# imironhead/ml_super_resolution

Measured on AMD Instinct MI355X. Metric: VDSR-20 training patches/sec (41x41, batch 256 per GPU); fwd HR megapixels/sec alongside, higher is better.
Workload: dtype f32; 1 GPU; BASELINE configs[2]: VDSR 20-layer 3x3x64 residual, RGB, batch 256x41x41 per GPU, fwd+bwd+TF-Adam, random-init weights; global_batch=256, patch=41, parallelism=dp1

## Files before the change

include/srx.h:

```cpp
#ifndef SRX_H_
#define SRX_H_

#include <stddef.h>
#include <stdint.h>

#ifdef __cplusplus
extern "C" {
#endif

typedef void* srx_stream_t;

typedef enum {
    SRX_OK = 0,
    SRX_ERR_BAD_ARG = -1,
    SRX_ERR_UNSUPPORTED = -2,
    SRX_ERR_WORKSPACE = -3,
    SRX_ERR_LAUNCH = -4,
    SRX_ERR_ALIGN = -5
} srx_status;

typedef enum { SRX_PAD_SAME = 0, SRX_PAD_VALID = 1 } srx_pad_mode;

typedef enum {
    SRX_ACT_NONE = 0,
// ... 18 lines not shown
} srx_conv_desc;

const char* srx_version(void);
const char* srx_last_error(void);

int srx_set_conv_path(int pipelined);

int srx_set_wgrad_path(int path);

int srx_conv_chain(const srx_conv_desc* d, int op, int in_act, int layers, const float* const* x, const float* const* w,
                   const float* const* bias, const float* const* aux, float* const* y, srx_stream_t stream);

int srx_conv_chain_supported(const srx_conv_desc* d, int op, int in_act);

int srx_set_chain(int on);

int srx_conv2d_precision_supported(const srx_conv_desc* d, int op);

size_t srx_conv2d_workspace_bytes(const srx_conv_desc* d, int op);

int srx_conv2d_fwd(const srx_conv_desc* d, const float* x, const float* w, const float* bias,
                   const float* skip, float* y, void* ws, size_t ws_bytes, srx_stream_t stream);

int srx_conv2d_bwd_data(const srx_conv_desc* d, const float* dpre, const float* w,
                        const float* x_in, int in_act, float* dx_out, void* ws, size_t ws_bytes,
                        srx_stream_t stream);

int srx_conv2d_bwd_data_acc(const srx_conv_desc* d, const float* dpre, const float* w, const float* dx_acc,
                            float* dx_out, void* ws, size_t ws_bytes, srx_stream_t stream);

// ... 163 lines not shown
```

ml_super_resolution_amd/_lib.py:

```python
import ctypes
import os

_HERE = os.path.dirname(os.path.abspath(__file__))
LIB_PATH = os.path.join(_HERE, 'libsrx.so')

SRX_OK = 0
PAD_SAME, PAD_VALID = 0, 1
ACT_NONE, ACT_RELU, ACT_TANH, ACT_LRELU, ACT_SIGMOID = 0, 1, 2, 3, 4
OP_FWD, OP_BWD_DATA, OP_BWD_FILTER = 0, 1, 2
PRECISION_FP32, PRECISION_BF16X3 = 0, 1
PRECISION_BY_NAME = {'highest': PRECISION_FP32, 'high': PRECISION_BF16X3}

ACT_BY_NAME = {None: ACT_NONE, 'none': ACT_NONE, 'relu': ACT_RELU, 'tanh': ACT_TANH,
               'lrelu': ACT_LRELU, 'leaky_relu': ACT_LRELU, 'sigmoid': ACT_SIGMOID}
PAD_BY_NAME = {'same': PAD_SAME, 'valid': PAD_VALID}

EXPORTS = [
    'srx_version', 'srx_last_error', 'srx_set_conv_path', 'srx_set_wgrad_path', 'srx_set_chain', 'srx_conv_chain', 'srx_conv_chain_supported', 'srx_conv2d_precision_supported', 'srx_conv2d_workspace_bytes', 'srx_conv2d_fwd',
    'srx_conv2d_bwd_data', 'srx_conv2d_bwd_filter', 'srx_conv2d_bwd_filter_partials', 'srx_conv2d_bwd_filter_reduce', 'srx_act_bwd', 'srx_depth_to_space',
    'srx_space_to_depth', 'srx_stream_copy', 'srx_mse_fwd_bwd', 'srx_l2_loss', 'srx_reduce_scratch_bytes',
    'srx_adam_tf_step', 'srx_adam_tf_step_dev', 'srx_momentum_clip_step', 'srx_rownorm_loss_fwd_bwd', 'srx_psnr', 'srx_ssim', 'srx_ssim_scratch_bytes', 'srx_saturate_u8', 'srx_affine', 'srx_u8_to_unit_float', 'srx_gaussian_blur', 'srx_resize_bilinear',
    'srx_upsample_nearest', 'srx_upsample_nearest_bwd', 'srx_add_relu_grad',
    'srx_conv2d_bwd_data_acc', 'srx_conv3x3_blocked', 'srx_conv3x3_blocked_bwd_filter_workspace_bytes', 'srx_conv3x3_blocked_bwd_filter',
    'srx_conv3x3_blocked_ex', 'srx_conv3x3_blocked_bwd_filter_ex_workspace_bytes', 'srx_conv3x3_blocked_bwd_filter_ex',
    'srx_espcn_forward', 'srx_espcn_forward_keep', 'srx_debug_poison_lds', 'srx_srcnn_forward', 'srx_maxpool2x2', 'srx_maxpool2x2_bwd', 'srx_maxpool2x2_bwd_masked', 'srx_subsample2', 'srx_subsample2_bwd',
    'srx_channel_blocks_to_nhwc', 'srx_nhwc_to_channel_blocks', 'srx_channel_normalize', 'srx_channel_normalize_bwd',
    'srx_extract_patches16', 'srx_texture_gram', 'srx_texture_gram_bwd', 'srx_pil_resample_ksize', 'srx_pil_resample_coeffs', 'srx_resample_u8', 'srx_u8_to_pm1', 'srx_log_loss', 'srx_vgg_preprocess', 'srx_add_scaled', 'srx_resize_bicubic_tf', 'srx_column_sums', 'srx_gemm_workspace_bytes', 'srx_gemm',
]


class SrxError(RuntimeError):
    pass

# ... 22 lines not shown
    if not os.path.exists(LIB_PATH):
        raise SrxError('libsrx.so not found at %s -- build it with `make -C %s` (or '
                       '__graft_entry__.build()); there is no CPU fallback' %
                       (LIB_PATH, os.path.join(_HERE, 'csrc')))
    import torch
    L = ctypes.CDLL(LIB_PATH)
    vp, sz, i, f = ctypes.c_void_p, ctypes.c_size_t, ctypes.c_int, ctypes.c_float
    dp = ctypes.POINTER(ConvDesc)
    L.srx_version.restype = ctypes.c_char_p
    L.srx_last_error.restype = ctypes.c_char_p
    L.srx_set_conv_path.argtypes = [i]
    L.srx_set_wgrad_path.argtypes = [i]
    L.srx_set_chain.argtypes = [i]
    L.srx_conv_chain_supported.argtypes = [dp, i, i]
    L.srx_conv_chain.argtypes = [dp, i, i, i, vp, vp, vp, vp, vp, vp]
    L.srx_conv2d_precision_supported.argtypes = [dp, i]
    L.srx_conv2d_workspace_bytes.argtypes = [dp, i]
    L.srx_conv2d_workspace_bytes.restype = sz
    L.srx_reduce_scratch_bytes.restype = sz
    L.srx_conv2d_fwd.argtypes = [dp, vp, vp, vp, vp, vp, vp, sz, vp]
    L.srx_conv2d_bwd_data.argtypes = [dp, vp, vp, vp, i, vp, vp, sz, vp]
    L.srx_conv2d_bwd_filter.argtypes = [dp, vp, vp, vp, vp, vp, f, vp, sz, vp]
    L.srx_conv2d_bwd_filter_partials.argtypes = [dp, vp, vp, vp, sz, ctypes.POINTER(ctypes.c_int), vp]
    L.srx_conv2d_bwd_filter_reduce.argtypes = [dp, vp, i, vp, vp, vp, f, vp]
    L.srx_act_bwd.argtypes = [vp, vp, vp, sz, i, vp]
    L.srx_depth_to_space.argtypes = [vp, vp, i, i, i, i, i, vp]
    L.srx_space_to_depth.argtypes = [vp, vp, i, i, i, i, i, vp]
    L.srx_stream_copy.argtypes = [vp, vp, sz, vp]
    L.srx_mse_fwd_bwd.argtypes = [vp, vp, sz, f, vp, i, vp, vp, vp]
    L.srx_l2_loss.argtypes = [vp, vp, sz, f, vp, i, vp, vp]
# ... 63 lines not shown
```

ml_super_resolution_amd/csrc/conv_kernels.hip.h:

```cpp
#pragma once
#include <hip/hip_runtime.h>
#include <stdint.h>
#include <type_traits>

namespace srx {

typedef float f32x4 __attribute__((ext_vector_type(4)));

enum { ACT_NONE = 0, ACT_RELU = 1, ACT_TANH = 2, ACT_LRELU = 3, ACT_SIGMOID = 4 };

struct ConvArgs {
    const float* x;
    const float* w;
    const float* bias;
    const float* skip;
    const float* mask;
    float* y;
    int N, H, W, OH, OW, Cin, Cout;
    int pad_t, pad_l;
    int TH, TW, NTX, RS;
    int units_total;
    int act, post_relu, mask_act;
    float inv_rs;
    int stagger;
// ... 15 lines not shown
    int units_total;
    float inv_rs;
    int stagger;
    int zero_slot;
    int stride;
    unsigned long long* trace;
};

constexpr int kChainMax = 32;
struct ChainPtrs {
    const float* x[kChainMax];
    const float* w[kChainMax];
    const float* bias[kChainMax];
    const float* aux[kChainMax];
    float* y[kChainMax];
    int L;
};

template <int CINP>
struct Lds {
    static constexpr int PS = (CINP == 4) ? 4 : CINP + 4;
};

__device__ __forceinline__ float srx_tanhf(float x) {
    const float ax = fabsf(x);
    const float x2 = ax * ax;
    float p = fmaf(x2, -0.006274174898862839f, 0.021071631461381912f);
    p = fmaf(x2, p, -0.053852297365665436f);
    p = fmaf(x2, p, 0.13332585990428925f);
    p = fmaf(x2, p, -0.33333316445350647f);
// ... 2396 lines not shown
        }
    }
    bsum += __shfl_xor(bsum, 16);
    bsum += __shfl_xor(bsum, 32);
    if (qpart == 0 && kq == 0 && co_ok) pw[(size_t)TAPS * a.Cin * a.Cout + co] = bsum;
}

template <int IMM>
__device__ __forceinline__ float dpre_fire_imm(__amdgpu_buffer_rsrc_t rsrc, int voff, int soff) {
    float b;
    asm volatile("buffer_load_dword %0, %1, %2, %3 offen offset:%4" : "=&a"(b) : "v"(voff), "s"(rsrc), "s"(soff), "n"(IMM) : "memory");
    return b;
}

template <int KH, int KW, int CINP, int NCH, int OWC>
__global__ __launch_bounds__(256, 1) void wgrad_rows_full_kernel(const WgradArgs a) {
    extern __shared__ __attribute__((aligned(16))) float lds[];
    constexpr int PS = Lds<CINP>::PS;
    constexpr int TAPS = KH * KW;
    constexpr int ROWS = TAPS * CINP;
    constexpr int Q = (ROWS + 63) / 64;
    constexpr int NQP = 4 / NCH;
    constexpr int QW = (Q + NQP - 1) / NQP;
    constexpr int TPP = CINP / 4, PPP = 256 / TPP;
    constexpr int SPR = OWC / 4;
    constexpr int THC = 3;
    constexpr int RSZ = OWC + 1;
    constexpr int COUTC = 64;
    constexpr int U = THC * SPR + 1;
    constexpr int JP = (RSZ + PPP - 1) / PPP;
    constexpr int NPASSES = (THC + KH - 1) * JP;
// ... 17 lines not shown
    char* ldsb = reinterpret_cast<char*>(lds);
    const int buf_bytes = (a.zero_slot + 4) * PS * 4;

    typedef __attribute__((address_space(3))) const f32x4 lds_f32x4;
    const int lds_base = (int)(uintptr_t)(__attribute__((address_space(3))) char*)ldsb;
    int xw[QW];
#pragma unroll
    for (int k = 0; k < QW; ++k) {
        const int q = qpart + k * NQP;
        int R = 64 * q + 4 * li;
        if (q >= Q || R >= ROWS) R = 0;
        const int tap = R / CINP, ci = R % CINP;
        xw[k] = lds_base + ((kq + (tap / KW) * RSZ + (tap % KW)) * PS + ci) * 4;
    }
    const int dX = kq * (RSZ - 1) * PS * 4;
    {
        const f32x4 z = {0.f, 0.f, 0.f, 0.f};
        for (int i = tid; i < 2 * buf_bytes / 16; i += 256) reinterpret_cast<f32x4*>(lds)[i] = z;
    }
    const int voff_lane = tid * 16;
    const int wl_lane = (sp * PS + 4 * c4) * 4;
    StageGeo SG;
    SG.JP1 = __builtin_amdgcn_readfirstlane(JP - 1);
    SG.rowfix_g = __builtin_amdgcn_readfirstlane((a.W - JP * PPP) * CINP * 4);
    SG.rowfix_l = __builtin_amdgcn_readfirstlane((RSZ - JP * PPP) * PS * 4);
    SG.m_first = uniform64(__ballot(sp >= a.pad_l));
    SG.m_last = uniform64(__ballot((JP - 1) * PPP + sp < RSZ));
    SG.m_row = SG.m_last; SG.m_mid = ~0ull;
    const int colb = 16 * COUTC;
    const int lane_b = (kq * COUTC + co_c) * 4;
    const int vb0 = lane_b, vb1 = lane_b + 4 * colb, vb2 = lane_b + 8 * colb;
// ... 181 lines not shown
#pragma unroll
        for (int g = 0; g < 4; ++g) {
#pragma unroll
            for (int r = 0; r < 4; ++r) {
                const int R = 64 * q + 4 * (4 * kq + r) + g;
                const int tap = R / CINP, ci = R % CINP;
                if (R < ROWS && ci < a.Cin && co_ok) pw[((size_t)tap * a.Cin + ci) * a.Cout + co] = acc[k][g][r];
            }
        }
    }
    bsum += __shfl_xor(bsum, 16);
    bsum += __shfl_xor(bsum, 32);
    if (qpart == 0 && kq == 0 && co_ok) pw[(size_t)TAPS * a.Cin * a.Cout + co] = bsum;
}

}
```

ml_super_resolution_amd/csrc/launchers.h:

```cpp
#pragma once
#include "conv_kernels.hip.h"

namespace srx {

struct ConvKey {
    int kh, kw, cinp, nch;
    bool wt;
};

bool launch_conv_k3c64(const ConvKey& k, const ConvArgs& a, int grid, size_t lds, hipStream_t s, hipError_t* err);
bool launch_conv_k3c32(const ConvKey& k, const ConvArgs& a, int grid, size_t lds, hipStream_t s, hipError_t* err);
bool launch_conv_c4(const ConvKey& k, const ConvArgs& a, int grid, size_t lds, hipStream_t s, hipError_t* err);
bool launch_conv_misc(const ConvKey& k, const ConvArgs& a, int grid, size_t lds, hipStream_t s, hipError_t* err);
bool launch_pipe_k3c64(const ConvKey& k, const ConvArgs& a, int grid, size_t lds, hipStream_t s, hipError_t* err);
bool launch_pipe_other(const ConvKey& k, const ConvArgs& a, int grid, size_t lds, hipStream_t s, hipError_t* err);
bool launch_wgrad_narrow(const ConvKey& k, const WgradArgs& a, int grid, hipStream_t s, hipError_t* err);
bool launch_conv_narrow(const ConvKey& k, const ConvArgs& a, hipStream_t s, hipError_t* err);
bool launch_conv_1x1(const ConvKey& k, const ConvArgs& a, long min_pixels, hipStream_t s, hipError_t* err);
bool launch_conv_rows3x3(const ConvKey& k, const ConvArgs& a, long min_pixels, hipStream_t s, hipError_t* err);
bool launch_conv_pack3(const ConvKey& k, const ConvArgs& a, long min_pixels, hipStream_t s, hipError_t* err);
bool launch_conv_kwrows(const ConvKey& k, const ConvArgs& a, long min_pixels, hipStream_t s, hipError_t* err);
bool launch_pipe_strip(const ConvKey& k, const ConvArgs& a, int grid, size_t lds, hipStream_t s, hipError_t* err);
bool launch_conv_generic(const ConvKey& k, const ConvArgs& a, int grid, size_t lds, hipStream_t s, hipError_t* err);
bool launch_wgrad(const ConvKey& k, const WgradArgs& a, int grid, size_t lds, hipStream_t s, hipError_t* err);
// ... 2 lines not shown
bool launch_wgrad_lin_pack3(const ConvKey& k, const WgradArgs& a, int grid, size_t lds, hipStream_t s, hipError_t* err);
bool launch_wgrad_lin_strip(const ConvKey& k, const WgradArgs& a, int grid, size_t lds, hipStream_t s, hipError_t* err);
bool launch_wgrad_pipe(const ConvKey& k, const WgradArgs& a, int grid, size_t lds, hipStream_t s, hipError_t* err);
bool launch_wgrad_kwcols(const ConvKey& k, const WgradArgs& a, int max_partials, long min_pixels, int* n_partials, hipStream_t s, hipError_t* err);
bool launch_wgrad_1x1(const ConvKey& k, const WgradArgs& a, int max_partials, int* n_partials, hipStream_t s, hipError_t* err);
bool launch_wgrad_rows_full(const ConvKey& k, const WgradArgs& a, int grid, size_t lds, hipStream_t s, hipError_t* err);
bool launch_wgrad_rows_strip(const ConvKey& k, const WgradArgs& a, int grid, size_t lds, hipStream_t s, hipError_t* err);
bool launch_wgrad_lin_pairs(const ConvKey& k, const WgradPairs& q, int grid, int pairs, bool strips, size_t lds, hipStream_t s, hipError_t* err);

__attribute__((weak)) hipError_t launch_conv_chain(bool wt, bool aux, const ConvArgs& a, const ChainPtrs& c, int grid, size_t lds, hipStream_t s);

hipError_t launch_reduce_partials(const float* part, int G, int stride, int wn, int cout, float* dw, float* dbias,
                                  const float* w, float wd, hipStream_t s);
hipError_t launch_reduce_partials_pairs(const float* part, int G, int stride, int wn, int cout, float* dw, float* dbias,
                                        int pairs, int cob, hipStream_t s);

template <typename K, typename A>
inline hipError_t launch_with_lds(K kernel, const A& a, int grid, size_t lds, hipStream_t s, int grid_y = 1) {
    static thread_local const void* configured[64];
    static thread_local int n_configured = 0;
    const void* fn = reinterpret_cast<const void*>(kernel);
    bool known = false;
    for (int i = 0; i < n_configured; ++i) known |= (configured[i] == fn);
    if (!known) {
        hipError_t e = hipFuncSetAttribute(fn, hipFuncAttributeMaxDynamicSharedMemorySize, 160 * 1024);
        if (e != hipSuccess) return e;
        if (n_configured < 64) configured[n_configured++] = fn;
    }
    hipLaunchKernelGGL(kernel, dim3(grid, grid_y), dim3(256), lds, s, a);
    return hipGetLastError();
// ... 93 lines not shown
```

ml_super_resolution_amd/csrc/srx_api.hip:

```cpp
#include <math.h>
#include <stdarg.h>
#include <atomic>
#include <stdio.h>
#include <stdlib.h>
#include <string.h>

#include "../../include/srx.h"
#include "elementwise.h"
#include "launchers.h"
#include "bf16x3.h"

using namespace srx;

namespace {

thread_local char g_err[512] = "";

struct Knobs {
    int pipe_default, narrow, wgrad_lin, wgrad_pipe, wgrad_pipe_strip, wgrad_rows_full, wgrad_1x1, wgrad_pack3, kwrows_min_pixels, big_route_min_pixels, strip_d2s, conv_1x1_min_pixels, pack3_dgrad;
    int chain;
    unsigned long long* trace;
    int dbg;
};
int env_int(const char* name, int dflt) { const char* e = getenv(name); return e ? atoi(e) : dflt; }
Knobs read_knobs() {
    Knobs k;
    k.pipe_default = env_int("SRX_PIPE", 1);
    k.narrow = env_int("SRX_NARROW", 1);
    k.wgrad_lin = env_int("SRX_WGRAD_LIN", 1);
    k.wgrad_pipe = env_int("SRX_WGRAD_PIPE", 1);
    k.wgrad_pipe_strip = env_int("SRX_WGRAD_PIPE_STRIP", 1);
    k.kwrows_min_pixels = env_int("SRX_KWROWS_MIN_PIXELS", 4096);
    k.big_route_min_pixels = env_int("SRX_BIG_ROUTE_MIN_PIXELS", 60000);
    k.conv_1x1_min_pixels = env_int("SRX_CONV_1X1_MIN_PIXELS", 100000);
    k.pack3_dgrad = env_int("SRX_PACK3_DGRAD", 1);
    k.strip_d2s = env_int("SRX_STRIP_D2S", 1);
    k.wgrad_rows_full = env_int("SRX_WGRAD_ROWS_FULL", 1);
    k.wgrad_1x1 = env_int("SRX_WGRAD_1X1", 1);
    k.wgrad_pack3 = env_int("SRX_WGRAD_PACK3", 1);
    k.chain = env_int("SRX_CHAIN", 1);
    k.trace = nullptr;
    k.dbg = 0;
#ifdef SRX_TRACE
    { const char* tp = getenv("SRX_TRACE_PTR"); k.trace = tp ? (unsigned long long*)strtoull(tp, nullptr, 0) : nullptr; }
    k.dbg = env_int("SRX_DBG", 0);
#endif
    return k;
}
const Knobs& knobs() { static const Knobs k = read_knobs(); return k; }

std::atomic<int> g_use_pipe{-1};
std::atomic<int> g_chain{-1};
int use_chain() { const int v = g_chain.load(std::memory_order_relaxed); return v < 0 ? (knobs().chain ? 1 : 0) : v; }
int use_pipe() { const int v = g_use_pipe.load(std::memory_order_relaxed); return v < 0 ? knobs().pipe_default : v; }
std::atomic<int> g_wgrad_path{-1};
int wgrad_path_default() { return !knobs().wgrad_lin ? 0 : ((knobs().wgrad_pipe || knobs().wgrad_pipe_strip) ? 2 : 1); }
int wgrad_path() { const int v = g_wgrad_path.load(std::memory_order_relaxed); return v < 0 ? wgrad_path_default() : v; }

int cu_count() {
    static std::atomic<int> cached[64];
    int dev = 0;
    if (hipGetDevice(&dev) != hipSuccess || dev < 0 || dev >= 64) { (void)hipGetLastError(); return 256; }
    int n = cached[dev].load(std::memory_order_relaxed);
    if (n > 0) return n;
    if (hipDeviceGetAttribute(&n, hipDeviceAttributeMultiprocessorCount, dev) != hipSuccess || n <= 0) {
        (void)hipGetLastError();
        n = 256;
    }
// ... 519 lines not shown
    memset(&a, 0, sizeof(a));
    a.x = dpre; a.w = w; a.bias = nullptr; a.skip = dx_acc; a.mask = x_in; a.y = dx_out;
    fill_conv_args(&a, p, d->N, OH, OW, d->Cout, d->Cin);
    a.act = SRX_ACT_NONE; a.post_relu = 0; a.mask_act = in_act;
    return dispatch_conv(p, true, a, (hipStream_t)stream);
}

static void wgrad_tile_for_linear_walk(const srx_conv_desc* d, Plan* p) {
    if (p->NTX != 1 || wgrad_path() < 1) return;
    const size_t slot_bytes = (size_t)((p->cinp == 4) ? 4 : p->cinp + 4) * 4;
    while (p->TH > 1 && p->lds_bytes + 4 * slot_bytes > 80 * 1024) {
        p->TH -= 1;
        p->lds_bytes = ((size_t)(p->TH + d->KH - 1) * p->RS + (d->KW - 1)) * slot_bytes;
    }
}

int srx_conv2d_bwd_filter_partials(const srx_conv_desc* d, const float* x, const float* dpre, void* ws, size_t ws_bytes,
                                   int* n_partials, srx_stream_t stream) {
    int rc = check_desc(d);
    if (rc) return rc;
    if (!x || !dpre || !n_partials) return fail(SRX_ERR_BAD_ARG, "null tensor pointer");
    if (!aligned16(x) || !aligned16(dpre)) return fail(SRX_ERR_ALIGN, "tensor base pointers must be 16-byte aligned");
    if (d->precision == SRX_PRECISION_BF16X3) {
        if ((rc = bf16x3_supported(d, SRX_OP_BWD_FILTER)) != SRX_OK) return rc;
        Bf3Plan bp;
        bf16x3_plan(d->N, d->H, d->W, max_grid(), true, &bp);
        const size_t need = (size_t)bp.grid * part_stride(d) * sizeof(float);
        if (!ws || ws_bytes < need) return fail(SRX_ERR_WORKSPACE, "bwd_filter needs %zu workspace bytes, got %zu", need, ws_bytes);
        if (!aligned16(ws)) return fail(SRX_ERR_ALIGN, "workspace must be 16-byte aligned");
        const hipError_t err = launch_wgrad3x3c64_bf16x3(x, dpre, (float*)ws, (int)part_stride(d), d->N, d->H, d->W, bp, (hipStream_t)stream);
// ... 35 lines not shown
    const bool lin_ok = use_lin && p.NTX == 1 && OW >= 4 && p.RS >= 8 && p.RS == d->W + pl && (long)p.TH * OW * d->Cout * 4 < (1L << 30) &&
                        (long)d->H * d->W * d->Cin * 4 < (1L << 31) - 4096;
    const size_t lin_lds = p.lds_bytes + 4 * (size_t)((p.cinp == 4) ? 4 : p.cinp + 4) * 4;
    const int use_wpipe = wpath >= 2 && knobs().wgrad_pipe;
    const int wppp = (p.cinp >= 16) ? 256 / (p.cinp / 4) : 256;
    int wgrid = p.grid;
    bool wdone = false;
    if (knobs().wgrad_1x1 && wpath >= 1 && !s2) {
        int n1 = 0;
        if (launch_wgrad_1x1(k, a, p.grid, &n1, s, &err)) { wdone = true; wgrid = n1; }
    }
    if (!wdone && knobs().big_route_min_pixels >= 0 && wpath >= 1 && !s2) {
        int n1 = 0;
        if (launch_wgrad_kwcols(k, a, p.grid, knobs().big_route_min_pixels, &n1, s, &err)) { wdone = true; wgrid = n1; }
    }
    if (!wdone && use_wpipe && knobs().wgrad_rows_full && lin_ok && d->KH == 3 && d->KW == 3 && d->Cin == 64 && d->Cout == 64 && OW == 41 && d->W == 41 &&
        pl == 1 && pt == 1 && p.RS == 42) {
        WgradArgs ap = a;
        ap.TH = 3;
        ap.zero_slot = (3 + 3) * 42 + 2;
        wgrid = p.grid < kPipeGrid ? p.grid : kPipeGrid;
        wdone = launch_wgrad_rows_full(k, ap, wgrid, 2 * (size_t)(ap.zero_slot + 4) * (64 + 4) * 4, s, &err);
        if (!wdone) wgrid = p.grid;
    }
    if (!wdone && use_wpipe && lin_ok && d->Cin == p.cinp && p.RS >= wppp && 2 * lin_lds <= 160 * 1024) {
        const int kWin = 14 * 4;
        int best_th = 0;
        double best_waste = 1e9;
        for (int th = p.TH; th >= 1; --th) {
            const long pos = (long)th * p.RS, padded = (pos + kWin - 1) / kWin * kWin;
            const double waste = (double)(padded - pos) / (double)pos;
            const bool fits = padded + 2L * p.RS + 6 <= (long)a.zero_slot + 4;
            if (fits && waste < best_waste - 1e-9) { best_waste = waste; best_th = th; }
        }
        if (best_th > 0 && best_waste <= 0.10) {
            WgradArgs ap = a;
            ap.TH = best_th;
// ... 37 lines not shown
    if (n_partials <= 0 || n_partials > kMaxGridLimit) return fail(SRX_ERR_BAD_ARG, "bad partial count %d", n_partials);
    const size_t wn = (size_t)d->KH * d->KW * d->Cin * d->Cout;
    hipError_t err = launch_reduce_partials((const float*)ws, n_partials, (int)part_stride(d), (int)wn, d->Cout, dw, dbias,
                                            w_for_decay, wd_scale, (hipStream_t)stream);
    if (err != hipSuccess) return fail(SRX_ERR_LAUNCH, "reduce launch failed: %s", hipGetErrorString(err));
    return SRX_OK;
}

int srx_conv2d_bwd_filter(const srx_conv_desc* d, const float* x, const float* dpre, float* dw, float* dbias,
                          const float* w_for_decay, float wd_scale, void* ws, size_t ws_bytes, srx_stream_t stream) {
    if (!dw) return fail(SRX_ERR_BAD_ARG, "null tensor pointer");
    int n = 0;
    const int rc = srx_conv2d_bwd_filter_partials(d, x, dpre, ws, ws_bytes, &n, stream);
    if (rc) return rc;
    return srx_conv2d_bwd_filter_reduce(d, ws, n, dw, dbias, w_for_decay, wd_scale, stream);
}

namespace {
void blocked_desc(srx_conv_desc* d, int N, int H, int W) {
    memset(d, 0, sizeof(*d));
    d->N = N; d->H = H; d->W = W; d->Cin = 64; d->Cout = 64; d->KH = 3; d->KW = 3; d->stride = 1; d->pad_mode = SRX_PAD_SAME;
}
int pairs_route(const srx_conv_desc* d, const Plan& p, int pairs, int* G, size_t* lin_lds) {
    *lin_lds = p.lds_bytes + 4 * (size_t)(p.cinp + 4) * 4;
    const bool common = wgrad_path() >= 1 && p.cinp == 64 && p.nch == 4 && d->W >= 4 && p.RS >= 8 && *lin_lds <= 80 * 1024 &&
                        (long)d->H * d->W * 64 * 4 < (1L << 31) - 4096;
    const bool lin_ok = common && p.NTX == 1 && p.RS == d->W + p.pad_l && (long)p.TH * d->W * 64 * 4 < (1L << 30);
    const int wppp = 256 / (64 / 4);
    const bool strip_ok = common && p.NTX > 1 && p.RS >= wppp && p.TW >= 4 && (d->W % p.TW == 0 || d->W % p.TW >= 4) &&
                          p.RS <= 3 * wppp && (long)d->H * d->W * 64 * 4 < (1L << 30);
// ... 316 lines not shown
```

ml_super_resolution_amd/csrc/wgrad_inst.hip:

```cpp
#include "launchers.h"
namespace srx {
__device__ __forceinline__ void reduce_partials_body(const float* __restrict__ part, int G, int stride, int wn, int n,
                                                     float* __restrict__ dw, float* __restrict__ dbias,
                                                     const float* __restrict__ w, float wd) {
    __shared__ f32x4 sh[16][17];
    const int c = threadIdx.x & 15, pg = threadIdx.x >> 4;
    const int j = blockIdx.x * 64 + 4 * c;
    f32x4 s = {0.f, 0.f, 0.f, 0.f};
    if (j < n) {
        const float* p = part + j;
        int g = pg;
        for (; g + 7 * 16 < G; g += 8 * 16) {
            f32x4 v[8];
#pragma unroll
            for (int i = 0; i < 8; ++i) v[i] = *reinterpret_cast<const f32x4*>(p + (size_t)(g + 16 * i) * stride);
#pragma unroll
            for (int i = 0; i < 8; ++i) s += v[i];
        }
        for (; g < G; g += 16) s += *reinterpret_cast<const f32x4*>(p + (size_t)g * stride);
    }
    sh[pg][c] = s;
    __syncthreads();
    if (pg == 0 && j < n) {
        f32x4 t = sh[0][c];
// ... 10 lines not shown
    }
}

__global__ __launch_bounds__(256) void reduce_partials_kernel(const float* __restrict__ part, int G, int stride,
                                                              int wn, int n, float* __restrict__ dw,
                                                              float* __restrict__ dbias, const float* __restrict__ w,
                                                              float wd) {
    reduce_partials_body(part, G, stride, wn, n, dw, dbias, w, wd);
}
__global__ __launch_bounds__(256) void reduce_partials_pairs_kernel(const float* __restrict__ part, int G, int stride,
                                                                    int wn, int n, float* __restrict__ dw,
                                                                    float* __restrict__ dbias, int cob) {
    const int pair = blockIdx.y;
    float* db = (dbias && pair < cob) ? dbias + (size_t)pair * (n - wn) : nullptr;
    reduce_partials_body(part + (size_t)pair * G * stride, G, stride, wn, n, dw + (size_t)pair * wn, db, nullptr, 0.f);
}

hipError_t launch_reduce_partials_pairs(const float* part, int G, int stride, int wn, int cout, float* dw, float* dbias,
                                        int pairs, int cob, hipStream_t s) {
    const int n = wn + cout;
    hipLaunchKernelGGL(reduce_partials_pairs_kernel, dim3((unsigned)((n + 63) / 64), (unsigned)pairs), dim3(256), 0, s, part, G,
                       stride, wn, n, dw, dbias, cob);
    return hipGetLastError();
}

hipError_t launch_reduce_partials(const float* part, int G, int stride, int wn, int cout, float* dw, float* dbias,
                                  const float* w, float wd, hipStream_t s) {
    const int n = wn + cout;
    hipLaunchKernelGGL(reduce_partials_kernel, dim3((unsigned)((n + 63) / 64)), dim3(256), 0, s, part, G, stride, wn, n,
                       dw, dbias, w, wd);
// ... 43 lines not shown
```

ml_super_resolution_amd/engine.py:

```python
import math
import os

import torch

from . import ops


class LayerSpec(object):

    def __init__(self, ksize, cin, cout, padding='same', act=None, scope=None):
        self.kh, self.kw = (ksize, ksize) if isinstance(ksize, int) else ksize
        self.cin, self.cout = cin, cout
        self.padding = padding.lower()
        self.act = act
        self.scope = scope

    @property
    def kernel_shape(self):
        return (self.kh, self.kw, self.cin, self.cout)

    def out_hw(self, h, w):
        if self.padding == 'same':
            return h, w
        return h - self.kh + 1, w - self.kw + 1
# ... 163 lines not shown
            j += 1
        return j

    def _dgrad_chain(self, acts):
        last = len(self.specs) - 1
        for hi in range(last - 1, 0, -1):
            s = self.specs[hi]
            lo = hi
            while (lo >= 1 and hi - lo < 32 and self.specs[lo].padding == s.padding and self.specs[lo - 1].act == self.specs[hi - 1].act and
                   tuple(acts[lo].shape) == tuple(acts[hi].shape) and self._chain_ok(lo, acts[lo].shape, ops._lib.OP_BWD_DATA)):
                lo -= 1
            if hi - lo >= 2:
                return lo + 1, hi
        return None

    def loss_and_backward(self, target, numel_global=None):
        if self._acts is None:
            raise RuntimeError('forward(keep=True) must run before loss_and_backward')
        acts = self._acts
        y = acts[-1]
        last = len(self.specs) - 1
        inv = 1.0 / (y.numel() if numel_global is None else numel_global)
        if self.loss_kind == 'rownorm':
            row_len = y.shape[1] * y.shape[2]
            dy = ops.rownorm_loss_fwd_bwd(y, target, row_len, self.loss, dpred=self._buf(('dy', 0), y.shape),
                                          norms=self._buf(('rownorms',), (y.numel() // row_len,)))
        else:
            dy = self._buf(('dy', 0), y.shape)
            ops.mse_fwd_bwd(y, target, self.loss, inv_numel=inv, accumulate=False, dpred=dy)
        if self.weight_decay:
            self.add_regulariser_loss()
        if self.specs[last].act is not None:
            dpre = ops.act_bwd(dy, y, self.specs[last].act, out=self._buf(('dpre_last',), y.shape))
        else:
            dpre = dy
        prec = self.layer_precision
        need = max(ops.bwd_filter_workspace_bytes(acts[i].shape, s.kernel_shape, s.padding, precision=prec[i])
                   for i, s in enumerate(self.specs))
        if self._ws is None or self._ws.numel() * 4 < need:
            self._step_graphs.clear()
            self._ws = torch.empty((need + 3) // 4, dtype=torch.float32, device=self.device)
        chain = self._dgrad_chain(acts)
        for i in range(last, -1, -1):
            s = self.specs[i]
            if chain is not None and chain[0] <= i <= chain[1]:
                lo, hi = chain
                if i == hi:
                    outs = [self._buf(('dpre_chain', k - 1), acts[k].shape) for k in range(hi, lo - 1, -1)]
                    ops.conv2d_bwd_data_chain([dpre] + outs[:-1], [self.kernel(k) for k in range(hi, lo - 1, -1)],
                                              [acts[k] for k in range(hi, lo - 1, -1)], outs, acts[hi].shape, s.padding,
                                              in_act=self.specs[hi - 1].act)
                    dpres = {hi: dpre}
                    for k in range(hi, lo - 1, -1):
                        dpres[k - 1] = outs[hi - k]
                ops.conv2d_bwd_filter(acts[i], dpres[i], s.kernel_shape, s.padding,
                                      w_for_decay=self.kernel(i) if self.weight_decay else None,
                                      wd_scale=self.weight_decay, dw=self.kernel(i, self.grads),
                                      dbias=self.bias(i, self.grads), workspace=self._ws, precision=prec[i])
                if i == lo:
                    dpre = dpres[lo - 1]
                continue
            ops.conv2d_bwd_filter(acts[i], dpre, s.kernel_shape, s.padding,
                                  w_for_decay=self.kernel(i) if self.weight_decay else None,
                                  wd_scale=self.weight_decay, dw=self.kernel(i, self.grads),
                                  dbias=self.bias(i, self.grads), workspace=self._ws, precision=prec[i])
            if i > 0:
                prev_act = self.specs[i - 1].act
                out = self._buf(('dx', i % 3, acts[i].shape[3]), acts[i].shape)
                dpre = ops.conv2d_bwd_data(dpre, self.kernel(i), acts[i].shape, s.padding,
                                           x_in=acts[i] if prev_act is not None else None, in_act=prev_act, out=out,
                                           precision=prec[i])
        if self.grad_hook is not None:
            self.grad_hook(self.grads)
        return self.loss

    def add_regulariser_loss(self):
        if self._decay_mask is None:
            self._decay_mask = torch.zeros_like(self.params)
            for k_off, kn, _, _ in self.slices:
                self._decay_mask[k_off:k_off + kn] = 1.0
        ops.l2_loss(self.params, self.weight_decay, self.loss, accumulate=True, mask=self._decay_mask)

    def adam_step(self, lr, beta1=0.9, beta2=0.999, eps=1e-8):
        if self.opt_m is None:
            self.opt_m = torch.zeros_like(self.params)
            self.opt_v = torch.zeros_like(self.params)
# ... 203 lines not shown
```

ml_super_resolution_amd/ops.py:

```python
import ctypes
import os

import torch

from . import _lib
from ._lib import ACT_BY_NAME, PAD_BY_NAME, ConvDesc, check
from ._lib import lib as _load_lib

_POISON_LDS = os.environ.get('SRX_POISON_LDS', '0') == '1'


def lib():
    L = _load_lib()
    if _POISON_LDS and torch.cuda.is_available():
        L.srx_debug_poison_lds(_stream())
    return L



def _stream():
    return ctypes.c_void_p(torch.cuda.current_stream().cuda_stream)


def _ptr(t):
# ... 151 lines not shown
    _chk(x, 'x'); _chk(dpre, 'dpre'); _chk(workspace, 'workspace')
    d = conv_desc(x.shape, w_shape, padding, precision=precision)
    n = ctypes.c_int(0)
    check(lib().srx_conv2d_bwd_filter_partials(ctypes.byref(d), _ptr(x), _ptr(dpre), _ptr(workspace), workspace.numel() * 4,
                                               ctypes.byref(n), _stream()), 'srx_conv2d_bwd_filter_partials')
    return n.value


def conv2d_bwd_filter_reduce(x_shape, w_shape, padding, workspace, n_partials, dw, dbias=None, w_for_decay=None, wd_scale=0.0,
                             precision='highest'):
    _chk(workspace, 'workspace'); _chk(dw, 'dw')
    d = conv_desc(x_shape, w_shape, padding, precision=precision)
    check(lib().srx_conv2d_bwd_filter_reduce(ctypes.byref(d), _ptr(workspace), int(n_partials), _ptr(dw), _ptr(dbias),
                                             _ptr(w_for_decay), float(wd_scale), _stream()), 'srx_conv2d_bwd_filter_reduce')
    return dw, dbias


def act_bwd(dy, y, act, out=None):
    _chk(dy, 'dy'); _chk(y, 'y')
    out = out if out is not None else torch.empty_like(dy)
    check(lib().srx_act_bwd(_ptr(dy), _ptr(y), _ptr(out), dy.numel(), ACT_BY_NAME[act], _stream()), 'srx_act_bwd')
    return out


def depth_to_space(x, r, out=None):
    _chk(x, 'x')
    N, H, W, D = x.shape
    if D % (r * r):
        raise ValueError('depth %d not divisible by r*r=%d' % (D, r * r))
    C = D // (r * r)
# ... 509 lines not shown
```

Measured before the change: 18940 patches/s.

## Chain weight-gradient partials across layers in one persistent kernel and batch reductions

Adds a persistent wgrad chain kernel that runs the 41-pixel-row weight-gradient body for every 64->64 3x3 layer of the dgrad chain in a single launch. It zeroes LDS only on the first layer and writes per-layer partials into a shared workspace. All layers' partial reductions, including weight decay and bias, are deferred to one multi-layer reduce launch at the end of backward. This removes per-layer launch overhead and reduce launches, at the cost of a larger workspace and a requirement that N be a multiple of the grid.

```diff
diff --git a/include/srx.h b/include/srx.h
--- a/include/srx.h
+++ b/include/srx.h
@@ -56,6 +56,19 @@
 int srx_conv_chain_supported(const srx_conv_desc* d, int op, int in_act);
 
 int srx_set_chain(int on);
+
+int srx_conv2d_bwd_filter_chain(const srx_conv_desc* d, int layers, const float* const* x, const float* const* dpre, void* ws,
+                                size_t ws_bytes, int* n_partials, srx_stream_t stream);
+
+int srx_conv2d_bwd_filter_chain_supported(const srx_conv_desc* d, int layers);
+
+size_t srx_conv2d_bwd_filter_chain_workspace_bytes(const srx_conv_desc* d, int layers);
+
+int srx_set_wgrad_chain(int on);
+
+int srx_conv2d_bwd_filter_reduce_layers(int layers, const srx_conv_desc* d, const void* const* ws, const int* n_partials,
+                                        float* const* dw, float* const* dbias, const float* const* w_for_decay, float wd_scale,
+                                        srx_stream_t stream);
 
 int srx_conv2d_precision_supported(const srx_conv_desc* d, int op);
 
diff --git a/ml_super_resolution_amd/_lib.py b/ml_super_resolution_amd/_lib.py
--- a/ml_super_resolution_amd/_lib.py
+++ b/ml_super_resolution_amd/_lib.py
@@ -16,7 +16,7 @@
 PAD_BY_NAME = {'same': PAD_SAME, 'valid': PAD_VALID}
 
 EXPORTS = [
-    'srx_version', 'srx_last_error', 'srx_set_conv_path', 'srx_set_wgrad_path', 'srx_set_chain', 'srx_conv_chain', 'srx_conv_chain_supported', 'srx_conv2d_precision_supported', 'srx_conv2d_workspace_bytes', 'srx_conv2d_fwd',
+    'srx_version', 'srx_last_error', 'srx_set_conv_path', 'srx_set_wgrad_path', 'srx_set_chain', 'srx_conv_chain', 'srx_conv_chain_supported', 'srx_conv2d_bwd_filter_chain', 'srx_conv2d_bwd_filter_chain_supported', 'srx_conv2d_bwd_filter_chain_workspace_bytes', 'srx_set_wgrad_chain', 'srx_conv2d_bwd_filter_reduce_layers', 'srx_conv2d_precision_supported', 'srx_conv2d_workspace_bytes', 'srx_conv2d_fwd',
     'srx_conv2d_bwd_data', 'srx_conv2d_bwd_filter', 'srx_conv2d_bwd_filter_partials', 'srx_conv2d_bwd_filter_reduce', 'srx_act_bwd', 'srx_depth_to_space',
     'srx_space_to_depth', 'srx_stream_copy', 'srx_mse_fwd_bwd', 'srx_l2_loss', 'srx_reduce_scratch_bytes',
     'srx_adam_tf_step', 'srx_adam_tf_step_dev', 'srx_momentum_clip_step', 'srx_rownorm_loss_fwd_bwd', 'srx_psnr', 'srx_ssim', 'srx_ssim_scratch_bytes', 'srx_saturate_u8', 'srx_affine', 'srx_u8_to_unit_float', 'srx_gaussian_blur', 'srx_resize_bilinear',
@@ -69,6 +69,12 @@
     L.srx_set_chain.argtypes = [i]
     L.srx_conv_chain_supported.argtypes = [dp, i, i]
     L.srx_conv_chain.argtypes = [dp, i, i, i, vp, vp, vp, vp, vp, vp]
+    L.srx_conv2d_bwd_filter_chain.argtypes = [dp, i, vp, vp, vp, sz, ctypes.POINTER(ctypes.c_int), vp]
+    L.srx_conv2d_bwd_filter_chain_supported.argtypes = [dp, i]
+    L.srx_conv2d_bwd_filter_chain_workspace_bytes.argtypes = [dp, i]
+    L.srx_conv2d_bwd_filter_chain_workspace_bytes.restype = sz
+    L.srx_set_wgrad_chain.argtypes = [i]
+    L.srx_conv2d_bwd_filter_reduce_layers.argtypes = [i, vp, vp, vp, vp, vp, vp, f, vp]
     L.srx_conv2d_precision_supported.argtypes = [dp, i]
     L.srx_conv2d_workspace_bytes.argtypes = [dp, i]
     L.srx_conv2d_workspace_bytes.restype = sz
diff --git a/ml_super_resolution_amd/csrc/conv_kernels.hip.h b/ml_super_resolution_amd/csrc/conv_kernels.hip.h
--- a/ml_super_resolution_amd/csrc/conv_kernels.hip.h
+++ b/ml_super_resolution_amd/csrc/conv_kernels.hip.h
@@ -53,6 +53,13 @@
     const float* bias[kChainMax];
     const float* aux[kChainMax];
     float* y[kChainMax];
+    int L;
+};
+
+struct WgradChainPtrs {
+    const float* x[kChainMax];
+    const float* dpre[kChainMax];
+    float* part[kChainMax];
     int L;
 };
 
@@ -2479,7 +2486,7 @@
 }
 
 template <int KH, int KW, int CINP, int NCH, int OWC>
-__global__ __launch_bounds__(256, 1) void wgrad_rows_full_kernel(const WgradArgs a) {
+__device__ __forceinline__ void wgrad_rows_full_body(const WgradArgs& a, bool lds_fill = true) {
     extern __shared__ __attribute__((aligned(16))) float lds[];
     constexpr int PS = Lds<CINP>::PS;
     constexpr int TAPS = KH * KW;
@@ -2527,7 +2534,7 @@
         xw[k] = lds_base + ((kq + (tap / KW) * RSZ + (tap % KW)) * PS + ci) * 4;
     }
     const int dX = kq * (RSZ - 1) * PS * 4;
-    {
+    if (lds_fill) {
         const f32x4 z = {0.f, 0.f, 0.f, 0.f};
         for (int i = tid; i < 2 * buf_bytes / 16; i += 256) reinterpret_cast<f32x4*>(lds)[i] = z;
     }
@@ -2739,4 +2746,9 @@
     if (qpart == 0 && kq == 0 && co_ok) pw[(size_t)TAPS * a.Cin * a.Cout + co] = bsum;
 }
 
-}
+template <int KH, int KW, int CINP, int NCH, int OWC>
+__global__ __launch_bounds__(256, 1) void wgrad_rows_full_kernel(const WgradArgs a) {
+    wgrad_rows_full_body<KH, KW, CINP, NCH, OWC>(a);
+}
+
+}
diff --git a/ml_super_resolution_amd/csrc/launchers.h b/ml_super_resolution_amd/csrc/launchers.h
--- a/ml_super_resolution_amd/csrc/launchers.h
+++ b/ml_super_resolution_amd/csrc/launchers.h
@@ -40,6 +40,19 @@
                                   const float* w, float wd, hipStream_t s);
 hipError_t launch_reduce_partials_pairs(const float* part, int G, int stride, int wn, int cout, float* dw, float* dbias,
                                         int pairs, int cob, hipStream_t s);
+
+constexpr int kReduceLayersMax = 40;
+struct ReduceLayers {
+    const float* part[kReduceLayersMax];
+    float* dw[kReduceLayersMax];
+    float* dbias[kReduceLayersMax];
+    const float* w[kReduceLayersMax];
+    int G[kReduceLayersMax], stride[kReduceLayersMax], wn[kReduceLayersMax], n[kReduceLayersMax];
+    int L;
+};
+__attribute__((weak)) hipError_t launch_reduce_partials_layers(const ReduceLayers& q, float wd, hipStream_t s);
+
+__attribute__((weak)) hipError_t launch_wgrad_chain(const WgradArgs& a, const WgradChainPtrs& c, int grid, size_t lds, hipStream_t s);
 
 template <typename K, typename A>
 inline hipError_t launch_with_lds(K kernel, const A& a, int grid, size_t lds, hipStream_t s, int grid_y = 1) {
diff --git a/ml_super_resolution_amd/csrc/srx_api.hip b/ml_super_resolution_amd/csrc/srx_api.hip
--- a/ml_super_resolution_amd/csrc/srx_api.hip
+++ b/ml_super_resolution_amd/csrc/srx_api.hip
@@ -18,7 +18,7 @@
 
 struct Knobs {
     int pipe_default, narrow, wgrad_lin, wgrad_pipe, wgrad_pipe_strip, wgrad_rows_full, wgrad_1x1, wgrad_pack3, kwrows_min_pixels, big_route_min_pixels, strip_d2s, conv_1x1_min_pixels, pack3_dgrad;
-    int chain;
+    int chain, wgrad_chain;
     unsigned long long* trace;
     int dbg;
 };
@@ -39,6 +39,7 @@
     k.wgrad_1x1 = env_int("SRX_WGRAD_1X1", 1);
     k.wgrad_pack3 = env_int("SRX_WGRAD_PACK3", 1);
     k.chain = env_int("SRX_CHAIN", 1);
+    k.wgrad_chain = env_int("SRX_WGRAD_CHAIN", 1);
     k.trace = nullptr;
     k.dbg = 0;
 #ifdef SRX_TRACE
@@ -52,6 +53,11 @@
 std::atomic<int> g_use_pipe{-1};
 std::atomic<int> g_chain{-1};
 int use_chain() { const int v = g_chain.load(std::memory_order_relaxed); return v < 0 ? (knobs().chain ? 1 : 0) : v; }
+std::atomic<int> g_wgrad_chain{-1};
+int use_wgrad_chain() {
+    const int v = g_wgrad_chain.load(std::memory_order_relaxed);
+    return use_chain() && (v < 0 ? (knobs().wgrad_chain ? 1 : 0) : v);
+}
 int use_pipe() { const int v = g_use_pipe.load(std::memory_order_relaxed); return v < 0 ? knobs().pipe_default : v; }
 std::atomic<int> g_wgrad_path{-1};
 int wgrad_path_default() { return !knobs().wgrad_lin ? 0 : ((knobs().wgrad_pipe || knobs().wgrad_pipe_strip) ? 2 : 1); }
@@ -601,6 +607,19 @@
         p->lds_bytes = ((size_t)(p->TH + d->KH - 1) * p->RS + (d->KW - 1)) * slot_bytes;
     }
 }
+
+static bool wgrad_rows_full_ok(const srx_conv_desc* d, const Plan& p, int pt, int pl, int OH, int OW) {
+    const int wpath = wgrad_path();
+    const bool lin_ok = wpath >= 1 && d->stride != 2 && p.NTX == 1 && OW >= 4 && p.RS >= 8 && p.RS == d->W + pl &&
+                        (long)p.TH * OW * d->Cout * 4 < (1L << 30) && (long)d->H * d->W * d->Cin * 4 < (1L << 31) - 4096;
+    return wpath >= 2 && knobs().wgrad_pipe && knobs().wgrad_rows_full && lin_ok && d->KH == 3 && d->KW == 3 && d->Cin == 64 &&
+           d->Cout == 64 && OW == 41 && d->W == 41 && pl == 1 && pt == 1 && p.RS == 42;
+}
+static void wgrad_rows_full_args(WgradArgs* ap) {
+    ap->TH = 3;
+    ap->zero_slot = (3 + 3) * 42 + 2;
+}
+static size_t wgrad_rows_full_lds(const WgradArgs& ap) { return 2 * (size_t)(ap.zero_slot + 4) * (64 + 4) * 4; }
 
 int srx_conv2d_bwd_filter_partials(const srx_conv_desc* d, const float* x, const float* dpre, void* ws, size_t ws_bytes,
                                    int* n_partials, srx_stream_t stream) {
@@ -666,13 +685,11 @@
         int n1 = 0;
         if (launch_wgrad_kwcols(k, a, p.grid, knobs().big_route_min_pixels, &n1, s, &err)) { wdone = true; wgrid = n1; }
     }
-    if (!wdone && use_wpipe && knobs().wgrad_rows_full && lin_ok && d->KH == 3 && d->KW == 3 && d->Cin == 64 && d->Cout == 64 && OW == 41 && d->W == 41 &&
-        pl == 1 && pt == 1 && p.RS == 42) {
+    if (!wdone && wgrad_rows_full_ok(d, p, pt, pl, OH, OW)) {
         WgradArgs ap = a;
-        ap.TH = 3;
-        ap.zero_slot = (3 + 3) * 42 + 2;
+        wgrad_rows_full_args(&ap);
         wgrid = p.grid < kPipeGrid ? p.grid : kPipeGrid;
-        wdone = launch_wgrad_rows_full(k, ap, wgrid, 2 * (size_t)(ap.zero_slot + 4) * (64 + 4) * 4, s, &err);
+        wdone = launch_wgrad_rows_full(k, ap, wgrid, wgrad_rows_full_lds(ap), s, &err);
         if (!wdone) wgrid = p.grid;
     }
     if (!wdone && use_wpipe && lin_ok && d->Cin == p.cinp && p.RS >= wppp && 2 * lin_lds <= 160 * 1024) {
@@ -740,6 +757,112 @@
     const int rc = srx_conv2d_bwd_filter_partials(d, x, dpre, ws, ws_bytes, &n, stream);
     if (rc) return rc;
     return srx_conv2d_bwd_filter_reduce(d, ws, n, dw, dbias, w_for_decay, wd_scale, stream);
+}
+
+namespace {
+int wgrad_chain_plan(const srx_conv_desc* d, int layers, WgradArgs* a, int* grid, size_t* lds) {
+    int rc = check_desc(d);
+    if (rc) return rc;
+    if (layers < 1) return fail(SRX_ERR_BAD_ARG, "wgrad chain: %d layers", layers);
+    if (layers > kChainMax) return fail(SRX_ERR_UNSUPPORTED, "wgrad chain: %d layers (at most %d)", layers, kChainMax);
+    if (!use_wgrad_chain()) return fail(SRX_ERR_UNSUPPORTED, "wgrad chain: switched off (srx_set_chain / SRX_CHAIN, srx_set_wgrad_chain / SRX_WGRAD_CHAIN)");
+    if (!launch_wgrad_chain) return fail(SRX_ERR_UNSUPPORTED, "wgrad chain: this build has no chain kernels");
+    if (d->precision != SRX_PRECISION_FP32) return fail(SRX_ERR_UNSUPPORTED, "wgrad chain: precision %d (exact fp32 only)", d->precision);
+    if (d->KH != 3 || d->KW != 3 || d->Cin != 64 || d->Cout != 64 || d->stride != 1 || d->pad_mode != SRX_PAD_SAME)
+        return fail(SRX_ERR_UNSUPPORTED, "wgrad chain: only 3x3 64->64 stride-1 SAME layers");
+    int pt, pl, OH, OW;
+    geometry(d, &pt, &pl, &OH, &OW);
+    Plan p;
+    rc = make_plan(d->N, d->H, d->W, OH, OW, d->Cin, d->Cout, d->KH, d->KW, pt, pl, &p);
+    if (rc) return rc;
+    wgrad_tile_for_linear_walk(d, &p);
+    if (!wgrad_rows_full_ok(d, p, pt, pl, OH, OW))
+        return fail(SRX_ERR_UNSUPPORTED, "wgrad chain: the layer is not on the 41-pixel-row route (wgrad_rows_full_kernel)");
+    *grid = p.grid < pipe_grid() ? p.grid : pipe_grid();
+    if (d->N % *grid) return fail(SRX_ERR_UNSUPPORTED, "wgrad chain: N %d is not a multiple of the grid %d", d->N, *grid);
+    memset(a, 0, sizeof(*a));
+    a->part_stride = (int)part_stride(d);
+    a->N = d->N; a->H = d->H; a->W = d->W; a->OH = OH; a->OW = OW; a->Cin = d->Cin; a->Cout = d->Cout;
+    a->pad_t = pt; a->pad_l = pl; a->TW = p.TW; a->NTX = p.NTX; a->RS = p.RS;
+    a->units_total = p.units_total; a->inv_rs = 1.0f / (float)p.RS;
+    a->stagger = stagger_sleeps(p);
+    a->stride = 1;
+    wgrad_rows_full_args(a);
+    a->trace = nullptr;
+    *lds = wgrad_rows_full_lds(*a);
+    return SRX_OK;
+}
+}
+
+int srx_set_wgrad_chain(int on) {
+    const int old = g_wgrad_chain.exchange(on < 0 ? -1 : (on ? 1 : 0), std::memory_order_relaxed);
+    return old < 0 ? (knobs().wgrad_chain ? 1 : 0) : old;
+}
+
+int srx_conv2d_bwd_filter_chain_supported(const srx_conv_desc* d, int layers) {
+    WgradArgs a;
+    int grid;
+    size_t lds;
+    return wgrad_chain_plan(d, layers, &a, &grid, &lds) == SRX_OK ? 1 : 0;
+}
+
+size_t srx_conv2d_bwd_filter_chain_workspace_bytes(const srx_conv_desc* d, int layers) {
+    WgradArgs a;
+    int grid;
+    size_t lds;
+    if (wgrad_chain_plan(d, layers, &a, &grid, &lds) != SRX_OK) return 0;
+    return (size_t)layers * grid * a.part_stride * sizeof(float);
+}
+
+int srx_conv2d_bwd_filter_chain(const srx_conv_desc* d, int layers, const float* const* x, const float* const* dpre, void* ws,
+                                size_t ws_bytes, int* n_partials, srx_stream_t stream) {
+    if (!x || !dpre || !n_partials) return fail(SRX_ERR_BAD_ARG, "null pointer array");
+    WgradArgs a;
+    int grid;
+    size_t lds;
+    const int rc = wgrad_chain_plan(d, layers, &a, &grid, &lds);
+    if (rc) return rc;
+    const size_t layer_floats = (size_t)grid * a.part_stride, need = (size_t)layers * layer_floats * sizeof(float);
+    if (!ws || ws_bytes < need) return fail(SRX_ERR_WORKSPACE, "bwd_filter_chain needs %zu workspace bytes, got %zu", need, ws_bytes);
+    if (!aligned16(ws)) return fail(SRX_ERR_ALIGN, "workspace must be 16-byte aligned");
+    WgradChainPtrs c;
+    memset(&c, 0, sizeof(c));
+    c.L = layers;
+    for (int l = 0; l < layers; ++l) {
+        if (!x[l] || !dpre[l]) return fail(SRX_ERR_BAD_ARG, "wgrad chain: null tensor pointer in layer %d", l);
+        if (!aligned16(x[l]) || !aligned16(dpre[l])) return fail(SRX_ERR_ALIGN, "tensor base pointers must be 16-byte aligned");
+        c.x[l] = x[l]; c.dpre[l] = dpre[l]; c.part[l] = (float*)ws + (size_t)l * layer_floats;
+    }
+    const hipError_t err = launch_wgrad_chain(a, c, grid, lds, (hipStream_t)stream);
+    if (err != hipSuccess) return fail(SRX_ERR_LAUNCH, "wgrad chain launch failed: %s", hipGetErrorString(err));
+    *n_partials = grid;
+    return SRX_OK;
+}
+
+int srx_conv2d_bwd_filter_reduce_layers(int layers, const srx_conv_desc* d, const void* const* ws, const int* n_partials,
+                                        float* const* dw, float* const* dbias, const float* const* w_for_decay, float wd_scale,
+                                        srx_stream_t stream) {
+    if (layers < 1 || layers > kReduceLayersMax) return fail(SRX_ERR_BAD_ARG, "reduce_layers: %d layers (1..%d)", layers, kReduceLayersMax);
+    if (!d || !ws || !n_partials || !dw) return fail(SRX_ERR_BAD_ARG, "null pointer array");
+    if (!launch_reduce_partials_layers) return fail(SRX_ERR_UNSUPPORTED, "reduce_layers: this build has no kernel units");
+    ReduceLayers q;
+    memset(&q, 0, sizeof(q));
+    q.L = layers;
+    for (int l = 0; l < layers; ++l) {
+        int rc = check_desc(&d[l]);
+        if (rc) return rc;
+        if (d[l].precision == SRX_PRECISION_BF16X3 && (rc = bf16x3_supported(&d[l], SRX_OP_BWD_FILTER)) != SRX_OK) return rc;
+        if (!ws[l] || !dw[l]) return fail(SRX_ERR_BAD_ARG, "reduce_layers: null tensor pointer in layer %d", l);
+        if (!aligned16(ws[l])) return fail(SRX_ERR_ALIGN, "workspace must be 16-byte aligned");
+        if (n_partials[l] <= 0 || n_partials[l] > kMaxGridLimit) return fail(SRX_ERR_BAD_ARG, "bad partial count %d", n_partials[l]);
+        const size_t wn = (size_t)d[l].KH * d[l].KW * d[l].Cin * d[l].Cout;
+        q.part[l] = (const float*)ws[l]; q.dw[l] = dw[l]; q.dbias[l] = dbias ? dbias[l] : nullptr;
+        q.w[l] = w_for_decay ? w_for_decay[l] : nullptr;
+        q.G[l] = n_partials[l]; q.stride[l] = (int)part_stride(&d[l]); q.wn[l] = (int)wn; q.n[l] = (int)wn + d[l].Cout;
+    }
+    const hipError_t err = launch_reduce_partials_layers(q, wd_scale, (hipStream_t)stream);
+    if (err != hipSuccess) return fail(SRX_ERR_LAUNCH, "reduce launch failed: %s", hipGetErrorString(err));
+    return SRX_OK;
 }
 
 namespace {
diff --git a/ml_super_resolution_amd/csrc/wgrad_chain.hip b/ml_super_resolution_amd/csrc/wgrad_chain.hip
--- /dev/null
+++ b/ml_super_resolution_amd/csrc/wgrad_chain.hip
@@ -0,0 +1,25 @@
+#include "launchers.h"
+namespace srx {
+
+__global__ __launch_bounds__(256, 1) void wgrad_chain_kernel(const WgradArgs a, const WgradChainPtrs c) {
+    for (int l = 0; l < c.L; ++l) {
+        WgradArgs al = a;
+        al.x = c.x[l]; al.dpre = c.dpre[l]; al.part = c.part[l];
+        asm volatile("" : "+s"(al.N), "+s"(al.H), "+s"(al.W), "+s"(al.OH), "+s"(al.OW), "+s"(al.Cin), "+s"(al.Cout));
+        asm volatile("" : "+s"(al.pad_t), "+s"(al.pad_l), "+s"(al.units_total), "+s"(al.zero_slot), "+s"(al.part_stride));
+        wgrad_rows_full_body<3, 3, 64, 4, 41>(al, l == 0);
+    }
+}
+
+hipError_t launch_wgrad_chain(const WgradArgs& a, const WgradChainPtrs& c, int grid, size_t lds, hipStream_t s) {
+    static thread_local bool configured = false;
+    if (!configured) {
+        const hipError_t e = hipFuncSetAttribute(reinterpret_cast<const void*>(wgrad_chain_kernel),
+                                                 hipFuncAttributeMaxDynamicSharedMemorySize, 160 * 1024);
+        if (e != hipSuccess) return e;
+        configured = true;
+    }
+    hipLaunchKernelGGL(wgrad_chain_kernel, dim3(grid), dim3(256), lds, s, a, c);
+    return hipGetLastError();
+}
+}
diff --git a/ml_super_resolution_amd/csrc/wgrad_inst.hip b/ml_super_resolution_amd/csrc/wgrad_inst.hip
--- a/ml_super_resolution_amd/csrc/wgrad_inst.hip
+++ b/ml_super_resolution_amd/csrc/wgrad_inst.hip
@@ -48,6 +48,18 @@
     const int pair = blockIdx.y;
     float* db = (dbias && pair < cob) ? dbias + (size_t)pair * (n - wn) : nullptr;
     reduce_partials_body(part + (size_t)pair * G * stride, G, stride, wn, n, dw + (size_t)pair * wn, db, nullptr, 0.f);
+}
+
+__global__ __launch_bounds__(256) void reduce_partials_layers_kernel(const ReduceLayers q, float wd) {
+    const int l = blockIdx.y;
+    reduce_partials_body(q.part[l], q.G[l], q.stride[l], q.wn[l], q.n[l], q.dw[l], q.dbias[l], q.w[l], wd);
+}
+
+hipError_t launch_reduce_partials_layers(const ReduceLayers& q, float wd, hipStream_t s) {
+    int nmax = 0;
+    for (int l = 0; l < q.L; ++l) nmax = q.n[l] > nmax ? q.n[l] : nmax;
+    hipLaunchKernelGGL(reduce_partials_layers_kernel, dim3((unsigned)((nmax + 63) / 64), (unsigned)q.L), dim3(256), 0, s, q, wd);
+    return hipGetLastError();
 }
 
 hipError_t launch_reduce_partials_pairs(const float* part, int G, int stride, int wn, int cout, float* dw, float* dbias,
diff --git a/ml_super_resolution_amd/engine.py b/ml_super_resolution_amd/engine.py
--- a/ml_super_resolution_amd/engine.py
+++ b/ml_super_resolution_amd/engine.py
@@ -201,6 +201,25 @@
                 return lo + 1, hi
         return None
 
+    def _wgrad_chain(self, acts, chain):
+        if chain is None or self.grad_hook is not None or len(self.specs) > 40:
+            return None
+        if any(p != 'highest' for p in self.layer_precision):
+            return None
+        lo, hi = chain
+        s = self.specs[lo]
+        if not ops.wgrad_chain_supported(acts[lo].shape, s.kernel_shape, hi - lo + 1, s.padding):
+            return None
+        off = _align4((ops.wgrad_chain_workspace_bytes(acts[lo].shape, s.kernel_shape, hi - lo + 1, s.padding) + 3) // 4)
+        regions = {}
+        for i, si in enumerate(self.specs):
+            if lo <= i <= hi:
+                continue
+            n = _align4((ops.bwd_filter_workspace_bytes(acts[i].shape, si.kernel_shape, si.padding) + 3) // 4)
+            regions[i] = (off, n)
+            off += n
+        return off * 4, 0, regions
+
     def loss_and_backward(self, target, numel_global=None):
         if self._acts is None:
             raise RuntimeError('forward(keep=True) must run before loss_and_backward')
@@ -222,12 +241,17 @@
         else:
             dpre = dy
         prec = self.layer_precision
-        need = max(ops.bwd_filter_workspace_bytes(acts[i].shape, s.kernel_shape, s.padding, precision=prec[i])
-                   for i, s in enumerate(self.specs))
+        chain = self._dgrad_chain(acts)
+        wchain = self._wgrad_chain(acts, chain)
+        if wchain is not None:
+            need = wchain[0]
+        else:
+            need = max(ops.bwd_filter_workspace_bytes(acts[i].shape, s.kernel_shape, s.padding, precision=prec[i])
+                       for i, s in enumerate(self.specs))
         if self._ws is None or self._ws.numel() * 4 < need:
             self._step_graphs.clear()
             self._ws = torch.empty((need + 3) // 4, dtype=torch.float32, device=self.device)
-        chain = self._dgrad_chain(acts)
+        pending = {}
         for i in range(last, -1, -1):
             s = self.specs[i]
             if chain is not None and chain[0] <= i <= chain[1]:
@@ -240,6 +264,16 @@
                     dpres = {hi: dpre}
                     for k in range(hi, lo - 1, -1):
                         dpres[k - 1] = outs[hi - k]
+                    if wchain is not None:
+                        n = ops.conv2d_bwd_filter_chain([acts[k] for k in range(lo, hi + 1)], [dpres[k] for k in range(lo, hi + 1)],
+                                                        s.kernel_shape, s.padding, self._ws)
+                        per = n * ops.part_stride(s.kernel_shape)
+                        for k in range(lo, hi + 1):
+                            pending[k] = (self._ws[wchain[1] + (k - lo) * per:wchain[1] + (k - lo + 1) * per], n)
+                if wchain is not None:
+                    if i == lo:
+                        dpre = dpres[lo - 1]
+                    continue
                 ops.conv2d_bwd_filter(acts[i], dpres[i], s.kernel_shape, s.padding,
                                       w_for_decay=self.kernel(i) if self.weight_decay else None,
                                       wd_scale=self.weight_decay, dw=self.kernel(i, self.grads),
@@ -247,16 +281,28 @@
                 if i == lo:
                     dpre = dpres[lo - 1]
                 continue
-            ops.conv2d_bwd_filter(acts[i], dpre, s.kernel_shape, s.padding,
-                                  w_for_decay=self.kernel(i) if self.weight_decay else None,
-                                  wd_scale=self.weight_decay, dw=self.kernel(i, self.grads),
-                                  dbias=self.bias(i, self.grads), workspace=self._ws, precision=prec[i])
+            if wchain is not None:
+                off, n = wchain[2][i]
+                part = self._ws[off:off + n]
+                pending[i] = (part, ops.conv2d_bwd_filter_partials(acts[i], dpre, s.kernel_shape, s.padding, part))
+            else:
+                ops.conv2d_bwd_filter(acts[i], dpre, s.kernel_shape, s.padding,
+                                      w_for_decay=self.kernel(i) if self.weight_decay else None,
+                                      wd_scale=self.weight_decay, dw=self.kernel(i, self.grads),
+                                      dbias=self.bias(i, self.grads), workspace=self._ws, precision=prec[i])
             if i > 0:
                 prev_act = self.specs[i - 1].act
                 out = self._buf(('dx', i % 3, acts[i].shape[3]), acts[i].shape)
                 dpre = ops.conv2d_bwd_data(dpre, self.kernel(i), acts[i].shape, s.padding,
                                            x_in=acts[i] if prev_act is not None else None, in_act=prev_act, out=out,
                                            precision=prec[i])
+        if wchain is not None:
+            order = range(len(self.specs))
+            ops.conv2d_bwd_filter_reduce_layers([acts[i].shape for i in order], [self.specs[i].kernel_shape for i in order],
+                                                [self.specs[i].padding for i in order], [pending[i][0] for i in order],
+                                                [pending[i][1] for i in order], [self.kernel(i, self.grads) for i in order],
+                                                [self.bias(i, self.grads) for i in order],
+                                                [self.kernel(i) for i in order] if self.weight_decay else None, self.weight_decay)
         if self.grad_hook is not None:
             self.grad_hook(self.grads)
         return self.loss
diff --git a/ml_super_resolution_amd/ops.py b/ml_super_resolution_amd/ops.py
--- a/ml_super_resolution_amd/ops.py
+++ b/ml_super_resolution_amd/ops.py
@@ -189,6 +189,51 @@
     check(lib().srx_conv2d_bwd_filter_reduce(ctypes.byref(d), _ptr(workspace), int(n_partials), _ptr(dw), _ptr(dbias),
                                              _ptr(w_for_decay), float(wd_scale), _stream()), 'srx_conv2d_bwd_filter_reduce')
     return dw, dbias
+
+
+def wgrad_chain_supported(x_shape, w_shape, layers, padding='same', precision='highest'):
+    d = conv_desc(x_shape, w_shape, padding, precision=precision)
+    return lib().srx_conv2d_bwd_filter_chain_supported(ctypes.byref(d), int(layers)) == 1
+
+
+def wgrad_chain_workspace_bytes(x_shape, w_shape, layers, padding='same'):
+    d = conv_desc(x_shape, w_shape, padding)
+    return int(lib().srx_conv2d_bwd_filter_chain_workspace_bytes(ctypes.byref(d), int(layers)))
+
+
+def set_wgrad_chain(on):
+    return lib().srx_set_wgrad_chain(int(on))
+
+
+def conv2d_bwd_filter_chain(xs, dpres, w_shape, padding, workspace):
+    _chk(workspace, 'workspace')
+    d = conv_desc(xs[0].shape, w_shape, padding)
+    for l in range(len(xs)):
+        _chk(xs[l], 'x'); _chk(dpres[l], 'dpre')
+        if tuple(xs[l].shape) != tuple(xs[0].shape) or tuple(dpres[l].shape) != tuple(out_shape(d)):
+            raise ValueError('conv2d_bwd_filter_chain: layer %d does not have the shape of layer 0' % l)
+    n = ctypes.c_int(0)
+    check(lib().srx_conv2d_bwd_filter_chain(ctypes.byref(d), len(xs), _ptr_array(xs), _ptr_array(dpres), _ptr(workspace),
+                                            workspace.numel() * 4, ctypes.byref(n), _stream()), 'srx_conv2d_bwd_filter_chain')
+    return n.value
+
+
+def part_stride(w_shape):
+    kh, kw, cin, cout = w_shape
+    return (kh * kw * cin * cout + cout + 3) // 4 * 4
+
+
+def conv2d_bwd_filter_reduce_layers(x_shapes, w_shapes, paddings, workspaces, n_partials, dws, dbiases, w_for_decay=None,
+                                    wd_scale=0.0, precisions=None):
+    L = len(x_shapes)
+    descs = (ConvDesc * L)(*[conv_desc(x_shapes[l], w_shapes[l], paddings[l],
+                                       precision=precisions[l] if precisions is not None else 'highest') for l in range(L)])
+    for l in range(L):
+        _chk(workspaces[l], 'workspace'); _chk(dws[l], 'dw'); _chk(dbiases[l], 'dbias')
+    counts = (ctypes.c_int * L)(*[int(n) for n in n_partials])
+    check(lib().srx_conv2d_bwd_filter_reduce_layers(L, descs, _ptr_array(workspaces), counts, _ptr_array(dws), _ptr_array(dbiases),
+                                                    None if w_for_decay is None else _ptr_array(w_for_decay), float(wd_scale),
+                                                    _stream()), 'srx_conv2d_bwd_filter_reduce_layers')
 
 
 def act_bwd(dy, y, act, out=None):
```

Measured after the change: 19090 patches/s (median of 6 runs). No clear change (+0.8%).
